# BadgerTechnologies/navigation

Measured on NVIDIA B200. Metric: ms per updateMap+inflation @4k^2 grid; DWA trajectories scored/sec, lower is better.
Workload: dtype u8

## Files before the change

navigation_b200/csrc/costmap.cu:

```cuda
#include <algorithm>
#include <chrono>
#include <cmath>
#include <cstddef>
#include <cstdlib>
#include <cstring>
#include <limits>
#include <memory>
#include <vector>

#include "costmap_kernels.cuh"
#include "inflate_propagate.cuh"
#include "mirror_kernels.cuh"

namespace navgpu {

struct Pt {
  double x, y;
};

static double dist2d(double x0, double y0, double x1, double y1) { return hypot(x1 - x0, y1 - y0); }
static double distance_to_line(double pX, double pY, double x0, double y0, double x1, double y1) {
  double A = pX - x0, B = pY - y0, C = x1 - x0, D = y1 - y0;
  double dot = A * C + B * D, len_sq = C * C + D * D, param = dot / len_sq;
  double xx, yy;
// ... 271 lines not shown
  const uint16_t* rank = nullptr;
  const uint8_t* cost = nullptr;
  int max_blocks = 0;
};

int propagate_max_blocks(int device, int R, int* out, size_t* smem_set) {
  const size_t smem = propagate_smem(R);
  if (smem > 200 * 1024) return fail(NAVGPU_ERR_UNSUPPORTED, "propagation tables for R=%d need %zu B of shared memory", R, smem);
  if (smem > *smem_set) {
    NAVGPU_CUDA(cudaFuncSetAttribute(k_inflate_propagate, cudaFuncAttributeMaxDynamicSharedMemorySize, (int)smem));
    *smem_set = smem;
  }
  int per_sm = 0, sms = 0;
  NAVGPU_CUDA(cudaOccupancyMaxActiveBlocksPerMultiprocessor(&per_sm, k_inflate_propagate, kPThreads, smem));
  NAVGPU_CUDA(cudaDeviceGetAttribute(&sms, cudaDevAttrMultiProcessorCount, device));
  if (per_sm < 1) return fail(NAVGPU_ERR_UNSUPPORTED, "k_inflate_propagate does not fit an SM for R=%d", R);
  *out = per_sm * sms;
  return NAVGPU_OK;
}

int launch_propagate(const UpdateArgs& a, const uint16_t* seeds, const PropBuffers& pb, cudaStream_t stream) {
  PropArgs pa;
  pa.master = a.master;
  pa.sx = a.sx; pa.sy = a.sy; pa.pitch = a.pitch;
  pa.win = a.win;
  pa.R = a.R;
  pa.seeds = reinterpret_cast<const uint32_t*>(seeds);
  pa.state = pb.state;
  pa.rank = pb.rank;
  pa.cost = pb.cost;
  pa.ctl = pb.ctl;
  pa.list[0] = pb.list[0];
  pa.list[1] = pb.list[1];
  const long long cells = (long long)a.pitch * a.sy;
  const int blocks = (int)std::max<long long>(1, std::min<long long>(cells / 8192, pb.max_blocks));
  NAVGPU_CUDA(cudaMemsetAsync(pb.ctl, 0, sizeof(PropCtl), stream));
  NAVGPU_CUDA(cudaMemsetAsync(reinterpret_cast<char*>(pb.ctl) + offsetof(PropCtl, kmin), 0xff, sizeof(pb.ctl->kmin), stream));
  void* args[] = {&pa};
  NAVGPU_CUDA(cudaLaunchCooperativeKernel((const void*)k_inflate_propagate, dim3(blocks), dim3(kPThreads), args,
                                          propagate_smem(a.R), stream));
  NAVGPU_LAUNCHED(1);
  return NAVGPU_OK;
}

struct TileFlags {
  unsigned* ready = nullptr;
  unsigned epoch = 0;
  unsigned long long* trace = nullptr;
  unsigned* done = nullptr;
  bool* handed_over = nullptr;
};
static_assert(kMirrorInflateTileW == kITX && kMirrorInflateTileH == kITY, "k_mirror_diff waits for k_inflate's tiles");

int launch_sweep(const UpdateArgs& a, uint16_t* seeds, cudaStream_t stream, bool force_generic, cudaEvent_t ev_mid = nullptr,
                 const PropBuffers* prop = nullptr, const TileFlags* flags = nullptr) {
  const int R = a.R;
  if ((R <= 31 && !force_generic) || (prop && R > 0)) {
    MergeSeedArgs m;
    m.master = a.master;
    m.sx = a.sx; m.sy = a.sy; m.pitch = a.pitch;
    m.def = a.def;
    m.do_reset = a.do_reset;
    m.win = a.win;
    m.ml = a.ml;
    m.R = R;
    m.seeds = seeds;
    m.early = a.early; m.ex0 = a.ex0; m.exn = a.exn; m.ey0 = a.ey0; m.eyn = a.eyn;
    m.obst_flag = a.obst_flag; m.obst_epoch = a.obst_epoch;
    m.trace = flags ? flags->trace : nullptr;
    m.lean = a.ml.n >= 1 && a.ml.n <= 2 && a.ml.policy[0] == NAVGPU_TRUE_OVERWRITE &&
             (a.ml.n == 1 || a.ml.policy[1] == NAVGPU_MAX || a.ml.policy[1] == NAVGPU_OVERWRITE) && !getenv("NAVGPU_NO_LEAN_MERGE");
    if (R > 0 && !seeds) return fail(NAVGPU_ERR_INVALID, "seed bitmask missing");
    dim3 block(kMSGroupsX, kMSRowsY);
    dim3 grid((a.pitch + kMSGroupsX * 16 - 1) / (kMSGroupsX * 16), (a.sy + kMSTileH - 1) / kMSTileH);
    const bool handover = flags && flags->ready && a.early && R > 0 && !(prop && R > 0) && !ev_mid;
    if (handover) { m.ready = flags->ready; m.epoch = flags->epoch; }
    if (a.ml.n > 0 || a.do_reset || R > 0) {
      NAVGPU_CUDA(launch_pdl(k_merge_seed, grid, block, 0, stream, m));
      NAVGPU_LAUNCHED(1);
    }
    if (ev_mid) cudaEventRecord(ev_mid, stream);
    if (prop && R > 0) return launch_propagate(a, seeds, *prop, stream);
    if (R > 0) {
      InflateArgs ia;
      ia.master = a.master;
      ia.sx = a.sx; ia.sy = a.sy; ia.pitch = a.pitch;
      ia.win = a.win;
      ia.R = R;
      ia.reach2 = a.reach2;
      ia.cost_d2 = a.cost_d2;
      ia.seeds = reinterpret_cast<const uint32_t*>(seeds);
      if (handover) {
        ia.ready = flags->ready; ia.epoch = flags->epoch; ia.ready_pitch = (int)grid.x;
        ia.done = flags->done;
        if (flags->handed_over) *flags->handed_over = flags->done != nullptr;
      }
      ia.trace = flags ? flags->trace : nullptr;
      dim3 igrid((a.sx + kITX - 1) / kITX, (a.sy + kITY - 1) / kITY);
      const int reach = (int)sqrtf((float)a.reach2 + 0.5f);
      ia.reach = reach;
      if (reach <= 12) NAVGPU_CUDA(launch_pdl(k_inflate<12>, igrid, dim3(kIThreads), 0, stream, ia));
      else if (reach <= 20) NAVGPU_CUDA(launch_pdl(k_inflate<20>, igrid, dim3(kIThreads), 0, stream, ia));
      else NAVGPU_CUDA(launch_pdl(k_inflate<31>, igrid, dim3(kIThreads), 0, stream, ia));
      NAVGPU_LAUNCHED(1);
    }
    return NAVGPU_OK;
  }
  size_t smem = update_costs_smem(R);
  if (smem > 200 * 1024) return fail(NAVGPU_ERR_UNSUPPORTED, "cell inflation radius %d needs %zu B of shared memory", R, smem);
  if (smem > 48 * 1024)
    NAVGPU_CUDA(cudaFuncSetAttribute(k_update_costs, cudaFuncAttributeMaxDynamicSharedMemorySize, (int)smem));
  dim3 grid((a.sx + kTX - 1) / kTX, (a.sy + kTY - 1) / kTY);
  k_update_costs<<<grid, kUpdateThreads, smem, stream>>>(a);
  NAVGPU_LAUNCHED(1);
  return NAVGPU_OK;
}

int ensure_seeds(uint16_t** seeds, size_t* cap, unsigned pitch, unsigned sy, cudaStream_t stream) {
  const size_t need = size_t(seed_pitch16(pitch)) * sy * sizeof(uint16_t);
  if (*seeds && need <= *cap) return NAVGPU_OK;
  if (*seeds) cudaFree(*seeds);
  *seeds = nullptr;
  NAVGPU_CUDA(cudaMalloc(seeds, need));
  NAVGPU_CUDA(cudaMemsetAsync(*seeds, 0, need, stream));
  *cap = need;
  return NAVGPU_OK;
}

int ensure_prop(navgpu_costmap* h, const Layer& L, PropBuffers* pb) {
  if (!h->d_prop_state) {
    NAVGPU_CUDA(cudaMalloc(&h->d_prop_state, 3 * h->bytes() * sizeof(uint32_t)));
    NAVGPU_CUDA(cudaMalloc(&h->d_prop_ctl, sizeof(PropCtl)));
  }
  NAVGPU_TRY(propagate_max_blocks(h->device, (int)L.tables.R, &h->prop_max_blocks, &h->prop_smem_set));
  pb->state = h->d_prop_state;
  pb->list[0] = h->d_prop_state + h->bytes();
  pb->list[1] = h->d_prop_state + 2 * h->bytes();
  pb->ctl = h->d_prop_ctl;
  pb->rank = L.d_rank;
  pb->cost = L.d_cost2d;
  pb->max_blocks = h->prop_max_blocks;
  return NAVGPU_OK;
}

struct EarlyBox {
  int on = 0, x0 = 0, xn = 0, y0 = 0, yn = 0;
  const unsigned* flag = nullptr;
  unsigned epoch = 0;
};

int launch_update(navgpu_costmap* h, const MergeLayers& ml, int do_reset, int R, const uint8_t* cost_d2, int reach2 = 0,
                  const Layer* infl = nullptr, const EarlyBox* early = nullptr) {
  UpdateArgs a;
  a.early = early && early->on && do_reset ? 1 : 0;
  a.ex0 = early ? early->x0 : 0; a.exn = early ? early->xn : 0; a.ey0 = early ? early->y0 : 0; a.eyn = early ? early->yn : 0;
  if (a.early && early->flag) { a.obst_flag = early->flag; a.obst_epoch = early->epoch; }
// ... 1341 lines not shown
```

navigation_b200/csrc/costmap_kernels.cuh:

```cuda
#pragma once

#include "common.cuh"

namespace navgpu {

__device__ __forceinline__ unsigned long long trace_now() {
  unsigned long long t;
  asm volatile("mov.u64 %0, %%globaltimer;" : "=l"(t));
  return t;
}
__device__ __forceinline__ void trace_start(unsigned long long* tr, int k) {
  if (tr && (threadIdx.x | threadIdx.y) == 0) atomicMin(&tr[2 * k], trace_now());
}
__device__ __forceinline__ void trace_end(unsigned long long* tr, int k) {
  if (tr && (threadIdx.x | threadIdx.y) == 0) atomicMax(&tr[2 * k + 1], trace_now());
}
constexpr int kCtaTraceMax = 4096;
__device__ __forceinline__ void trace_cta(unsigned long long* tr, int kernel, int cta, int slot) {
  if (tr && (threadIdx.x | threadIdx.y) == 0 && cta < kCtaTraceMax) {
    unsigned long long* rec = tr + 16 + 8 * ((size_t)kernel * kCtaTraceMax + cta);
    rec[slot] = trace_now();
    if (slot == 0) {
      unsigned smid;
      asm volatile("mov.u32 %0, %%smid;" : "=r"(smid));
// ... 1042 lines not shown
  if (R > 0) {
    const int nwords = bits_pitch / 4;
    for (int item = tid; item < rows * kTX; item += kUpdateThreads) {
      const int row = item / kTX, tx = item - row * kTX;
      const uint32_t* wrow = reinterpret_cast<const uint32_t*>(bits + row * bits_pitch);
      const int p = HX + tx;
      auto word = [&](int i) -> uint32_t { return (i < 0 || i >= nwords) ? 0u : wrow[i]; };
      auto window32 = [&](int q) -> uint32_t {
        const int wi = q >> 5, sh = q & 31;
        return __funnelshift_r(word(wi), word(wi + 1), sh);
      };
      int best = 255;
      for (int base = 0; base <= R; base += 32) {
        const uint32_t right = window32(p + base);
        const uint32_t left = window32(p - base - 31);
        int d = 255;
        if (right) d = base + (__ffs(right) - 1);
        if (left) d = min(d, base + __clz(left));
        if (d != 255) { best = d; break; }
      }
      hx[item] = (uint8_t)(best <= R ? best : 255);
    }
    __syncthreads();

    const int tx = tid & (kTX - 1), half = tid / kTX;
    const int R2 = R * R;
    for (int r = half * (kTY / 2); r < (half + 1) * (kTY / 2); ++r) {
      int best = 0x7fffffff;
      const uint8_t* col = hx + (r + R) * kTX + tx;
      for (int dy = -R; dy <= R; ++dy) {
        const int h = col[dy * kTX];
        const int d2 = (h == 255) ? 0x7fffffff : h * h + dy * dy;
        best = min(best, d2);
      }
      if (best <= R2) {
        uint8_t* cell = tile + r * kTX + tx;
        *cell = inflate_combine(*cell, table[best]);
      }
    }
    __syncthreads();
  }

  for (int item = tid; item < kTX * kTY / 16; item += kUpdateThreads) {
    const int r = item / (kTX / 16), c = (item - r * (kTX / 16)) * 16;
    const int y = ty0 + r, x = tx0 + c;
    if (y < (int)a.sy && x < (int)a.pitch)
      *reinterpret_cast<uint4*>(a.master + (size_t)y * a.pitch + x) = *reinterpret_cast<const uint4*>(tile + r * kTX + c);
  }
}


constexpr int kMSGroupsX = 16, kMSRowsY = 16, kMSRowIters = 2, kMSSubTiles = 2;
constexpr int kMSTileH = kMSRowsY * kMSRowIters * kMSSubTiles;
static_assert(128 + 2 * 31 <= 256, "k_inflate: one thread per region row");
static_assert(kMSGroupsX * 16 == (int)kMarkTileW && kMSRowsY * kMSRowIters == (int)kMarkTileH, "MergeLayers::used tile");
constexpr int kITX = 64, kITY = 128, kIThreads = 256, kIMaxRows = kITY + 2 * 31;
constexpr int kIMaskWords = (kIMaxRows + 32 + 70 + 31) / 32 + 1;
constexpr int kISparseRows = 12;
constexpr uint32_t kH2Inf = 0x3000;

__host__ __device__ inline unsigned seed_pitch16(unsigned pitch) { return pitch / 16 + 4; }

struct MergeSeedArgs {
  uint8_t* master;
  unsigned sx, sy, pitch;
  uint8_t def;
  int do_reset;
  const DevWindow* win;
  MergeLayers ml;
  int R;
  uint16_t* seeds;
  int early = 0, ex0 = 0, exn = 0, ey0 = 0, eyn = 0;
  const unsigned* obst_flag = nullptr;
  unsigned obst_epoch = 0;
  unsigned* ready = nullptr;
  unsigned epoch = 0;
  unsigned long long* trace = nullptr;
  int lean = 0;
};

__device__ __forceinline__ uint32_t inc4(uint32_t x) {
  return ((x & 0x7f7f7f7fu) + 0x01010101u) ^ (x & 0x80808080u);
}

__device__ __forceinline__ uint32_t merge4(uint32_t m, uint32_t v, int policy) {
  switch (policy) {
    case NAVGPU_TRUE_OVERWRITE: return v;
    case NAVGPU_OVERWRITE: {
      const uint32_t vn = __vcmpeq4(v, 0xffffffffu);
      return (m & vn) | (v & ~vn);
    }
    case NAVGPU_MAX: {
      const uint32_t take = __vcmpltu4(inc4(m), inc4(v));
      return (v & take) | (m & ~take);
    }
    case NAVGPU_ADDITION: {
      const uint32_t vn = __vcmpeq4(v, 0xffffffffu), mn = __vcmpeq4(m, 0xffffffffu);
      uint32_t s = __vaddus4(m, v);
      const uint32_t ge = __vcmpgeu4(s, 0xfdfdfdfdu);
      s = (ge & 0xfcfcfcfcu) | (s & ~ge);
      const uint32_t r = (mn & v) | (~mn & s);
      return (vn & m) | (~vn & r);
    }
    default: return m;
  }
}

__device__ __forceinline__ uint4 merge16(uint4 m, uint4 v, int policy) {
  switch (policy) {
// ... 191 lines not shown
      trace_end(a.trace, 1);
      trace_cta(a.trace, 0, blockIdx.y * gridDim.x + blockIdx.x, 2);
      if (a.trace && touched && (threadIdx.x | threadIdx.y) == 0) atomicMax(&a.trace[6], trace_now());
      if (a.ready) {
        __syncthreads();
        if ((threadIdx.x | threadIdx.y) == 0)
          asm volatile("st.release.gpu.u32 [%0], %1;" ::"l"(a.ready + blockIdx.y * gridDim.x + blockIdx.x), "r"(a.epoch) : "memory");
      }
      if ((blockIdx.x | blockIdx.y) == 0) cudaGridDependencySynchronize();
      return;
    }
  } else {
    cudaGridDependencySynchronize();
    w = *a.win;
  }
  trace_cta(a.trace, 0, blockIdx.y * gridDim.x + blockIdx.x, 1);
  if (!w.valid) return;
  const int R = a.R;
  const int my = R > 0 ? 3 * R + kITY : 0, mx = R > 0 ? 2 * R + kITX + 32 : 0;
  if (bx0 >= w.xn + mx || bx0 + kW <= w.x0 - mx || by0 >= w.yn + my || by0 + kH <= w.y0 - my) return;
  const int sx0 = max(0, w.x0 - R), sxn = min((int)a.sx, w.xn + R);
  const int sy0 = max(0, w.y0 - R), syn = min((int)a.sy, w.yn + R);
  const int x = bx0 + threadIdx.x * 16;
  if (a.lean && bx0 >= w.x0 && bx0 + kW <= w.xn && by0 >= w.y0 && by0 + kH <= w.yn) {
    merge_seed_lean<false>(a, x, by0);
  } else {
    for (int sub = 0; sub < kMSSubTiles; ++sub) {
      constexpr int kSH = kMSRowsY * kMSRowIters;
      const int sy_0 = by0 + sub * kSH;
      if (sy_0 >= (int)a.sy || sy_0 >= w.yn + my || sy_0 + kSH <= w.y0 - my) continue;
      const bool interior = bx0 >= w.x0 && bx0 + kW <= w.xn && sy_0 >= w.y0 && sy_0 + kSH <= w.yn;
      unsigned used_mask = 0xffffffffu;
      for (int l = 0; l < a.ml.n; ++l)
        if (a.ml.used[l] && a.ml.used[l][(blockIdx.y * kMSSubTiles + sub) * gridDim.x + blockIdx.x] == 0) used_mask &= ~(1u << l);
      if (interior) {
        merge_seed_items<true>(a, w, x, sy_0, sx0, sxn, sy0, syn, used_mask);
      } else if (x < (int)a.pitch) {
        merge_seed_items<false>(a, w, x, sy_0, sx0, sxn, sy0, syn, used_mask);
      }
    }
  }
  trace_end(a.trace, 1);
  trace_cta(a.trace, 0, blockIdx.y * gridDim.x + blockIdx.x, 2);
  if (a.trace && a.early && bx0 < a.exn && bx0 + kW > a.ex0 && by0 < a.eyn && by0 + kH > a.ey0 && (threadIdx.x | threadIdx.y) == 0)
    atomicMax(&a.trace[6], trace_now());
  if (a.ready) {
    __syncthreads();
    if ((threadIdx.x | threadIdx.y) == 0)
      asm volatile("st.release.gpu.u32 [%0], %1;" ::"l"(a.ready + blockIdx.y * gridDim.x + blockIdx.x), "r"(a.epoch) : "memory");
  }
  if (a.early && (blockIdx.x | blockIdx.y) == 0) cudaGridDependencySynchronize();
}

struct Dy2Table {
  uint32_t v[8 + 2 * 31][8];
  constexpr Dy2Table() : v() {
    for (int p = 0; p < 8 + 2 * 31; ++p)
      for (int k = 0; k < 8; ++k) v[p][k] = (uint32_t)((p - 31 - k) * (p - 31 - k)) * 0x10001u;
  }
};
__constant__ Dy2Table c_dy2 = Dy2Table();

__device__ __forceinline__ int smem_fetch_add(int* p, int v) {
  int old;
  asm volatile("atom.shared.add.s32 %0, [%1], %2;" : "=r"(old) : "r"((unsigned)__cvta_generic_to_shared(p)), "r"(v) : "memory");
  return old;
}

__device__ __forceinline__ uint32_t ldg_u16(unsigned long long addr) {
  uint32_t v;
  asm volatile("ld.global.u16 %0, [%1];" : "=r"(v) : "l"(addr) : "memory");
  return v;
}
__device__ __forceinline__ void stg_u16(unsigned long long addr, uint32_t v) {
  asm volatile("st.global.u16 [%0], %1;" ::"l"(addr), "r"(v) : "memory");
}

struct InflateArgs {
  uint8_t* master;
  unsigned sx, sy, pitch;
  const DevWindow* win;
  int R;
  int reach2;
  int reach;
  const uint8_t* cost_d2;
  const uint32_t* seeds;
  const unsigned* ready = nullptr;
  unsigned epoch = 0;
  int ready_pitch = 0;
  unsigned* done = nullptr;
  unsigned long long* trace = nullptr;
};

template <int RMAX>
__device__ __forceinline__ void inflate_tile(const InflateArgs& a) {
  constexpr int kRows = kITY + 2 * RMAX;
  __shared__ __align__(16) uint32_t pbits[kRows * 4];
  __shared__ __align__(16) uint32_t h2[kRows * (kITX / 2)];
  uint32_t* const sbits = h2;
  __shared__ uint32_t rowmask[kIMaskWords];
  __shared__ uint32_t dupmask[kIMaskWords];
  __shared__ __align__(4) uint8_t canon[(kRows + 3) & ~3];
  __shared__ uint8_t rowlist[kRows];
  __shared__ int n_seeded;
  __shared__ int next_group;
  __shared__ __align__(16) uint8_t table[((RMAX + 1) * (RMAX + 1) + 1 + 15) & ~15];
  const int tx0 = blockIdx.x * kITX, ty0 = blockIdx.y * kITY;
  const unsigned* my_flag = nullptr;
  unsigned flag_seen = 0;
  cudaTriggerProgrammaticLaunchCompletion();
  trace_start(a.trace, 2);
  trace_cta(a.trace, 1, blockIdx.y * gridDim.x + blockIdx.x, 0);
  if (a.ready) {
    constexpr int kMW = kMSGroupsX * 16, kMH = kMSTileH;
    const int mx0 = max(0, tx0 - 32) / kMW, mx1 = min((int)a.pitch - 1, tx0 + kITX + 31) / kMW;
    const int my0 = max(0, ty0 - a.R) / kMH, my1 = min((int)a.sy - 1, ty0 + kITY + a.R - 1) / kMH;
    const int nx = mx1 - mx0 + 1, n = nx * (my1 - my0 + 1);
    if ((int)threadIdx.x < n) {
      my_flag = a.ready + (my0 + (int)threadIdx.x / nx) * a.ready_pitch + mx0 + (int)threadIdx.x % nx;
      asm volatile("ld.acquire.gpu.u32 %0, [%1];" : "=r"(flag_seen) : "l"(my_flag) : "memory");
    }
  }
  {
    const int zw = (a.reach2 + 1) >> 2;
    for (int i = threadIdx.x; i <= zw; i += kIThreads) {
      uint32_t v = reinterpret_cast<const uint32_t*>(a.cost_d2)[i];
      if (i == zw) v &= ~(0xffu << (8 * ((a.reach2 + 1) & 3)));
      reinterpret_cast<uint32_t*>(table)[i] = v;
    }
  }
  if (a.ready) {
    if (my_flag) {
      while (flag_seen != a.epoch) {
        __nanosleep(32);
        asm volatile("ld.acquire.gpu.u32 %0, [%1];" : "=r"(flag_seen) : "l"(my_flag) : "memory");
      }
    }
    __syncthreads();
    if (a.trace && threadIdx.x == 0) {
      atomicMin(&a.trace[7], trace_now());
      atomicMax(&a.trace[8], trace_now());
    }
    trace_cta(a.trace, 1, blockIdx.y * gridDim.x + blockIdx.x, 1);
  } else {
    cudaGridDependencySynchronize();
    const DevWindow w = *a.win;
    trace_cta(a.trace, 1, blockIdx.y * gridDim.x + blockIdx.x, 1);
    if (!w.valid) return;
    const int R = a.R;
    if (tx0 >= w.xn + 2 * R || tx0 + kITX <= w.x0 - 2 * R || ty0 >= w.yn + 2 * R || ty0 + kITY <= w.y0 - 2 * R) return;
  }
  const int R = a.reach;
  const int rows = kITY + 2 * R;
  const int tid = threadIdx.x, lane = tid & 31, warp = tid >> 5;
  const unsigned sp32 = seed_pitch16(a.pitch) / 2;

  int any = 0;
  {
    constexpr int NI = (kRows * 4 + kIThreads - 1) / kIThreads;
    uint32_t v[NI];
#pragma unroll
    for (int k = 0; k < NI; ++k) {
      const int i = tid + k * kIThreads, gy = ty0 - R + (i >> 2);
      v[k] = 0;
      if (i < rows * 4 && gy >= 0 && gy < (int)a.sy) v[k] = __ldcg(&a.seeds[(size_t)gy * sp32 + (tx0 >> 5) + (i & 3)]);
    }
    if (tid < kIMaskWords) rowmask[tid] = dupmask[tid] = 0;
    if (tid == 0) n_seeded = next_group = 0;
#pragma unroll
    for (int k = 0; k < NI; ++k) {
      const int i = tid + k * kIThreads;
      if (i < rows * 4) sbits[i] = v[k];
      any |= v[k] != 0;
    }
  }
  if (!__syncthreads_or(any)) {
    trace_end(a.trace, 2);
    trace_cta(a.trace, 1, blockIdx.y * gridDim.x + blockIdx.x, 2);
    return;
  }
  trace_cta(a.trace, 1, blockIdx.y * gridDim.x + blockIdx.x, 4);

  {
    const uint4* sb4 = reinterpret_cast<const uint4*>(sbits);
    auto pruned = [&](int r) -> uint4 {
      uint4 c = sb4[r];
      if ((c.x | c.y | c.z | c.w) != 0 && r > 0 && r + 1 < rows) {
        const uint4 u = sb4[r - 1], d = sb4[r + 1];
        const uint32_t kx = (c.x << 1) & ((c.x >> 1) | (c.y << 31)) & u.x & d.x;
        const uint32_t ky = ((c.y << 1) | (c.x >> 31)) & ((c.y >> 1) | (c.z << 31)) & u.y & d.y;
        const uint32_t kz = ((c.z << 1) | (c.y >> 31)) & ((c.z >> 1) | (c.w << 31)) & u.z & d.z;
        const uint32_t kw = ((c.w << 1) | (c.z >> 31)) & (c.w >> 1) & u.w & d.w;
        c.x &= ~kx; c.y &= ~ky; c.z &= ~kz; c.w &= ~kw;
      }
      c.x &= ~(0xffffffffu >> R);
      c.w &= (1u << R) - 1u;
      return c;
    };
    const int r = tid;
    bool seeded = false, dup = false;
    if (r < rows) {
      const uint4 k = pruned(r);
      reinterpret_cast<uint4*>(pbits)[r] = k;
      seeded = (k.x | k.y | k.z | k.w) != 0;
      if (seeded && r > 0) {
        const uint4 p = pruned(r - 1);
        dup = k.x == p.x && k.y == p.y && k.z == p.z && k.w == p.w;
      }
    }
    const uint32_t sm = __ballot_sync(0xffffffffu, seeded), dm = __ballot_sync(0xffffffffu, dup);
    const uint32_t lm = sm & ~dm;
    int base = 0;
    if (lane == 0 && sm) {
      rowmask[warp + 1] = sm;
      dupmask[warp + 1] = dm;
      if (lm) base = smem_fetch_add(&n_seeded, __popc(lm));
    }
    base = __shfl_sync(0xffffffffu, base, 0);
    if (seeded && !dup) rowlist[base + __popc(lm & ((1u << lane) - 1u))] = (uint8_t)r;
  }
  __syncthreads();
  trace_cta(a.trace, 1, blockIdx.y * gridDim.x + blockIdx.x, 5);

  {
    if (tid < rows) {
      int qq = warp;
      uint32_t z = ~dupmask[warp + 1] & (0xffffffffu >> (31 - lane));
      while (z == 0) z = ~dupmask[--qq + 1];
      canon[tid] = (uint8_t)(32 * qq + 31 - __clz(z));
    }
    const int n_rows_listed = n_seeded;
    for (int li = warp; li < n_rows_listed; li += kIThreads / 32) {
      const int r = rowlist[li];
      const uint4 W = reinterpret_cast<const uint4*>(pbits)[r];
      const uint32_t A = lane < 16 ? W.x : W.y, B = lane < 16 ? W.y : W.z, C = lane < 16 ? W.z : W.w;
      uint32_t packed = 0;
#pragma unroll
      for (int c = 0; c < 2; ++c) {
        const int sh = (2 * lane + c) & 31;
        const uint32_t right = __funnelshift_r(B, C, sh);
        const uint32_t left = __funnelshift_rc(A, B, sh + 1);
        int d = 64;
        if (right) d = __ffs(right) - 1;
        if (left) d = min(d, __clz(left));
        const uint32_t hh = d <= R ? (uint32_t)(d * d) : kH2Inf;
        packed |= hh << (16 * c);
      }
      h2[r * (kITX / 2) + lane] = packed;
    }
  }
  __syncthreads();
  trace_cta(a.trace, 1, blockIdx.y * gridDim.x + blockIdx.x, 6);

  const uint32_t R2x2 = (uint32_t)a.reach2 * 0x10001u;
  const int x = tx0 + 2 * lane;
  const bool xok = x < (int)a.sx;
  const uint32_t keep_hi = x + 1 >= (int)a.sx ? 0xff00u : 0u;
  const bool edge_tile = tx0 + kITX > (int)a.sx || ty0 + kITY > (int)a.sy;
  for (;;) {
    int g = 0;
    if (lane == 0) g = smem_fetch_add(&next_group, 1);
    g = __shfl_sync(0xffffffffu, g, 0);
    if (g >= kITY / 8) break;
    const int yr0 = g * 8;
    uint32_t acc[8];
#pragma unroll
    for (int k = 0; k < 8; ++k) acc[k] = 0x7fff7fffu;
    {
      constexpr int NJ = 8 + 2 * RMAX, NW = (NJ + 31) / 32, NB = (NJ + 7) / 8;
      const uint32_t* hb = h2 + lane;
      const uint8_t* cn = canon + yr0 + R;
      const int p0 = yr0 + R - RMAX + 32;
      const int wi = p0 >> 5, sh = p0 & 31;
      uint32_t mw[NW];
      uint32_t anyrow = 0;
      int nrows = 0;
#pragma unroll
      for (int q = 0; q < NW; ++q) {
        mw[q] = __funnelshift_r(rowmask[wi + q], rowmask[wi + q + 1], sh);
        if (q == NW - 1 && (NJ & 31) != 0) mw[q] &= (1u << (NJ & 31)) - 1u;
        const uint32_t dw = __funnelshift_r(dupmask[wi + q], dupmask[wi + q + 1], sh);
        constexpr int kBelow = RMAX + 8;
        const uint32_t below = 32 * q >= kBelow ? 0xffffffffu : (32 * q + 32 <= kBelow ? 0u : 0xffffffffu << (kBelow & 31));
        uint32_t drop = below & dw;
        if (q == 0) drop |= ((1u << RMAX) - 1u) & (dw >> 1);
        mw[q] &= ~drop;
        anyrow |= mw[q];
        nrows += __popc(mw[q]);
      }
      if (anyrow == 0) continue;
      if (nrows <= kISparseRows) {
#pragma unroll
        for (int q = 0; q < NW; ++q) {
          uint32_t m = mw[q];
          while (m) {
            const int j = __ffs(m) - 1 + 32 * q - RMAX;
            m &= m - 1;
            const uint32_t hh = hb[cn[j] * (kITX / 2)];
            const uint4* dq = reinterpret_cast<const uint4*>(c_dy2.v[j + 31]);
            const uint4 qa = dq[0], qb = dq[1];
            acc[0] = __viaddmin_u16x2(hh, qa.x, acc[0]);
            acc[1] = __viaddmin_u16x2(hh, qa.y, acc[1]);
            acc[2] = __viaddmin_u16x2(hh, qa.z, acc[2]);
            acc[3] = __viaddmin_u16x2(hh, qa.w, acc[3]);
            acc[4] = __viaddmin_u16x2(hh, qb.x, acc[4]);
            acc[5] = __viaddmin_u16x2(hh, qb.y, acc[5]);
            acc[6] = __viaddmin_u16x2(hh, qb.z, acc[6]);
            acc[7] = __viaddmin_u16x2(hh, qb.w, acc[7]);
          }
        }
      } else {
#pragma unroll
        for (int c = 0; c < NB; ++c) {
          const uint32_t bits8 = (mw[c >> 2] >> ((c & 3) * 8)) & 0xffu;
          if (bits8 == 0) continue;
#pragma unroll
          for (int b = 0; b < 8; ++b) {
            const int j = 8 * c + b - RMAX;
            if (j > 7 + RMAX) continue;
            if (bits8 & (1u << b)) {
              const uint32_t hh = hb[cn[j] * (kITX / 2)];
#pragma unroll
              for (int k = 0; k < 8; ++k) {
                const int dy = j - k;
                if (dy >= -RMAX && dy <= RMAX) acc[k] = __viaddmin_u16x2(hh, (uint32_t)(dy * dy) * 0x10001u, acc[k]);
              }
            }
          }
        }
      }
    }
    const uint32_t out_of_reach = R2x2 + 0x10001u;
    if (edge_tile) {
      const int kmax = xok ? min(8, (int)a.sy - (ty0 + yr0)) : 0;
#pragma unroll
      for (int k = 0; k < 8; ++k)
        if (k >= kmax) acc[k] = 0x7fff7fffu;
    }
    unsigned long long prow = (unsigned long long)__cvta_generic_to_global(a.master + ((size_t)(ty0 + yr0) * a.pitch + x));
    asm volatile("" : "+l"(prow));
    const uint32_t keep_hi4 = keep_hi * 0x10001u;
#pragma unroll
    for (int half = 0; half < 2; ++half) {
      uint32_t d2[4], cur[4];
#pragma unroll
      for (int q = 0; q < 4; ++q) {
        const int k = 4 * half + q;
        d2[q] = __vminu2(acc[k], out_of_reach);
        cur[q] = 0;
        if (d2[q] != out_of_reach) cur[q] = ldg_u16(prow + (unsigned long long)((uint32_t)k * a.pitch));
      }
      if (d2[0] == out_of_reach && d2[1] == out_of_reach && d2[2] == out_of_reach && d2[3] == out_of_reach) continue;
      uint32_t old4[2], out[2];
#pragma unroll
      for (int pr = 0; pr < 2; ++pr) {
        const uint32_t da = d2[2 * pr], db = d2[2 * pr + 1];
        const uint32_t c = ((uint32_t)table[da & 0xffffu] | ((uint32_t)table[da >> 16] << 8) |
                            ((uint32_t)table[db & 0xffffu] << 16) | ((uint32_t)table[db >> 16] << 24)) & ~keep_hi4;
        old4[pr] = cur[2 * pr] | (cur[2 * pr + 1] << 16);
        out[pr] = __vmaxu4(old4[pr], c);
        d2[2 * pr] = c;
      }
      if ((__vcmpeq4(old4[0], 0xffffffffu) | __vcmpeq4(old4[1], 0xffffffffu)) != 0) {
#pragma unroll
        for (int pr = 0; pr < 2; ++pr) {
          const uint32_t c = d2[2 * pr];
          out[pr] -= __vcmpeq4(old4[pr], 0xffffffffu) & __vcmpgeu4(c, 0xfdfdfdfdu) & ~c;
        }
      }
#pragma unroll
      for (int pr = 0; pr < 2; ++pr) {
        const int k = 4 * half + 2 * pr;
        const uint32_t diff = out[pr] ^ old4[pr];
        if (diff & 0xffffu) stg_u16(prow + (unsigned long long)((uint32_t)k * a.pitch), out[pr]);
        if (diff >> 16) stg_u16(prow + (unsigned long long)((uint32_t)(k + 1) * a.pitch), out[pr] >> 16);
      }
    }
  }
  trace_end(a.trace, 2);
  trace_cta(a.trace, 1, blockIdx.y * gridDim.x + blockIdx.x, 2);
}

template <int RMAX>
__global__ void __launch_bounds__(kIThreads, 8) k_inflate(InflateArgs a) {
  inflate_tile<RMAX>(a);
  if (a.ready && (blockIdx.x | blockIdx.y) == 0) cudaGridDependencySynchronize();
  if (a.done) {
    __syncthreads();
    if (threadIdx.x == 0)
      asm volatile("st.release.gpu.u32 [%0], %1;" ::"l"(a.done + blockIdx.y * gridDim.x + blockIdx.x), "r"(a.epoch) : "memory");
  }
}

inline size_t update_costs_smem(int R) {
  const int HX = (R + 7) & ~7;
  const int groups = (kTX + 2 * HX) / 8;
  const int rows = kTY + 2 * R;
  const int bits_pitch = (groups + 3) & ~3;
  return (size_t)kTX * kTY + ((rows * bits_pitch + 15) & ~15) + (size_t)rows * kTX + (size_t)R * R + 1 + 16;
}

}
```

navigation_b200/csrc/mirror_kernels.cuh:

```cuda
#pragma once

#include "common.cuh"

namespace navgpu {

constexpr int kMirrorTileW = 128, kMirrorTileH = 16;
constexpr int kMirrorTileBytes = kMirrorTileW * kMirrorTileH;
constexpr int kMirrorWarps = 8;

struct MirrorCtl {
  unsigned n_changed;
  unsigned n_staged;
  DevWindow win;
  unsigned seq;
};

struct MirrorArgs {
  const uint8_t* master;
  uint8_t* shadow;
  unsigned sx, sy, pitch;
  unsigned tiles_x, tiles_y;
  unsigned capacity;
  uint8_t* stage;
  unsigned* stage_tile;
  unsigned* counters;
  MirrorCtl* ctl;
  const DevWindow* win;
  DevWindow* dirty;
  int all;
  int hx0, hxn, hy0, hyn;
  unsigned tx0, ty0, tw, th;
  uint8_t* host_direct;
  unsigned host_pitch;
  unsigned seq;
  const unsigned* inflate_done = nullptr;
  unsigned inflate_epoch = 0;
  int inflate_pitch = 0;
};
constexpr int kMirrorInflateTileW = 64, kMirrorInflateTileH = 128;

__device__ __forceinline__ void mirror_wait_word(const unsigned* p, unsigned want) {
  unsigned seen;
  for (;;) {
    asm volatile("ld.acquire.gpu.u32 %0, [%1];" : "=r"(seen) : "l"(p) : "memory");
    if (seen == want) break;
    __nanosleep(100);
  }
}

__device__ __forceinline__ bool group_differs(const uint4& a, const uint4& b, int n_valid) {
  if (n_valid >= 16) return ((a.x ^ b.x) | (a.y ^ b.y) | (a.z ^ b.z) | (a.w ^ b.w)) != 0;
  const uint32_t d[4] = {a.x ^ b.x, a.y ^ b.y, a.z ^ b.z, a.w ^ b.w};
  uint32_t any = 0;
#pragma unroll
  for (int k = 0; k < 4; ++k) {
    const int nb = min(4, max(0, n_valid - 4 * k));
    const uint32_t mask = nb >= 4 ? 0xffffffffu : ((1u << (8 * nb)) - 1u);
    any |= d[k] & mask;
  }
  return any != 0;
}

__global__ void __launch_bounds__(kMirrorWarps * 32) k_mirror_diff(MirrorArgs a) {
  __shared__ bool s_last;
  const int lane = threadIdx.x & 31, warp = threadIdx.x >> 5;
  if (a.inflate_done) {
    if (lane == 0) mirror_wait_word(a.inflate_done, a.inflate_epoch);
    __syncwarp();
  } else {
    cudaGridDependencySynchronize();
  }
  const unsigned local = blockIdx.x * kMirrorWarps + warp;
  const unsigned n_tiles = a.tiles_x * a.tiles_y;
  const unsigned tile = local < a.tw * a.th ? (a.ty0 + local / a.tw) * a.tiles_x + a.tx0 + local % a.tw : n_tiles;
  int rx0 = 0, rxn = (int)a.sx, ry0 = 0, ryn = (int)a.sy;
  if (!a.all) {
    const DevWindow d = *a.dirty;
    if (d.valid) {
      rx0 = max(d.x0, a.hx0); rxn = min(d.xn, a.hxn); ry0 = max(d.y0, a.hy0); ryn = min(d.yn, a.hyn);
    } else {
      rxn = ryn = 0;
    }
  }
  const unsigned tx_ = tile % a.tiles_x, ty_ = tile / a.tiles_x;
  const bool in_region = (int)(tx_ * kMirrorTileW) < rxn && (int)((tx_ + 1) * kMirrorTileW) > rx0 &&
                         (int)(ty_ * kMirrorTileH) < ryn && (int)((ty_ + 1) * kMirrorTileH) > ry0;
  if (tile < n_tiles && in_region) {
    const unsigned tx = tx_, ty = ty_;
    if (a.inflate_done) {
      if (lane < kMirrorTileW / kMirrorInflateTileW) {
        const int ix = (int)(tx * kMirrorTileW) / kMirrorInflateTileW + lane, iy = (int)(ty * kMirrorTileH) / kMirrorInflateTileH;
        if (ix < a.inflate_pitch) mirror_wait_word(a.inflate_done + iy * a.inflate_pitch + ix, a.inflate_epoch);
// ... 69 lines not shown
```

Measured before the change: 0.04098.

## Widen inflate tiles to 128 columns with four columns per lane

Doubles the k_inflate tile width to 128 and the block to 512 threads. Each lane now handles four columns, with uint2 h2 loads and u32 global read-modify-writes in place of u16. Row groups shrink from 8 to 4 rows, and h2 moves to dynamic shared memory with an opt-in attribute. The aim is to cut halo overhead per tile and make the memory accesses wider, at the cost of more shared memory per block, lower occupancy (launch bounds 4), an extra __syncthreads, and changed handover tile granularity for the mirror kernel.

```diff
diff --git a/navigation_b200/csrc/costmap.cu b/navigation_b200/csrc/costmap.cu
--- a/navigation_b200/csrc/costmap.cu
+++ b/navigation_b200/csrc/costmap.cu
@@ -347,6 +347,18 @@
 };
 static_assert(kMirrorInflateTileW == kITX && kMirrorInflateTileH == kITY, "k_mirror_diff waits for k_inflate's tiles");
 
+int allow_inflate_smem() {
+  static std::atomic<bool> done_for_device[64] = {};
+  int dev = 0;
+  NAVGPU_CUDA(cudaGetDevice(&dev));
+  if (dev >= 0 && dev < 64 && done_for_device[dev].load(std::memory_order_acquire)) return NAVGPU_OK;
+  NAVGPU_CUDA(cudaFuncSetAttribute(k_inflate<12>, cudaFuncAttributeMaxDynamicSharedMemorySize, (int)inflate_h2_bytes(12)));
+  NAVGPU_CUDA(cudaFuncSetAttribute(k_inflate<20>, cudaFuncAttributeMaxDynamicSharedMemorySize, (int)inflate_h2_bytes(20)));
+  NAVGPU_CUDA(cudaFuncSetAttribute(k_inflate<31>, cudaFuncAttributeMaxDynamicSharedMemorySize, (int)inflate_h2_bytes(31)));
+  if (dev >= 0 && dev < 64) done_for_device[dev].store(true, std::memory_order_release);
+  return NAVGPU_OK;
+}
+
 int launch_sweep(const UpdateArgs& a, uint16_t* seeds, cudaStream_t stream, bool force_generic, cudaEvent_t ev_mid = nullptr,
                  const PropBuffers* prop = nullptr, const TileFlags* flags = nullptr) {
   const int R = a.R;
@@ -394,9 +406,10 @@
       dim3 igrid((a.sx + kITX - 1) / kITX, (a.sy + kITY - 1) / kITY);
       const int reach = (int)sqrtf((float)a.reach2 + 0.5f);
       ia.reach = reach;
-      if (reach <= 12) NAVGPU_CUDA(launch_pdl(k_inflate<12>, igrid, dim3(kIThreads), 0, stream, ia));
-      else if (reach <= 20) NAVGPU_CUDA(launch_pdl(k_inflate<20>, igrid, dim3(kIThreads), 0, stream, ia));
-      else NAVGPU_CUDA(launch_pdl(k_inflate<31>, igrid, dim3(kIThreads), 0, stream, ia));
+      NAVGPU_TRY(allow_inflate_smem());
+      if (reach <= 12) NAVGPU_CUDA(launch_pdl(k_inflate<12>, igrid, dim3(kIThreads), inflate_h2_bytes(12), stream, ia));
+      else if (reach <= 20) NAVGPU_CUDA(launch_pdl(k_inflate<20>, igrid, dim3(kIThreads), inflate_h2_bytes(20), stream, ia));
+      else NAVGPU_CUDA(launch_pdl(k_inflate<31>, igrid, dim3(kIThreads), inflate_h2_bytes(31), stream, ia));
       NAVGPU_LAUNCHED(1);
     }
     return NAVGPU_OK;
diff --git a/navigation_b200/csrc/costmap_kernels.cuh b/navigation_b200/csrc/costmap_kernels.cuh
--- a/navigation_b200/csrc/costmap_kernels.cuh
+++ b/navigation_b200/csrc/costmap_kernels.cuh
@@ -1118,9 +1118,12 @@
 
 constexpr int kMSGroupsX = 16, kMSRowsY = 16, kMSRowIters = 2, kMSSubTiles = 2;
 constexpr int kMSTileH = kMSRowsY * kMSRowIters * kMSSubTiles;
-static_assert(128 + 2 * 31 <= 256, "k_inflate: one thread per region row");
 static_assert(kMSGroupsX * 16 == (int)kMarkTileW && kMSRowsY * kMSRowIters == (int)kMarkTileH, "MergeLayers::used tile");
-constexpr int kITX = 64, kITY = 128, kIThreads = 256, kIMaxRows = kITY + 2 * 31;
+constexpr int kITX = 128, kITY = 128, kIThreads = 512, kIMaxRows = kITY + 2 * 31;
+constexpr int kISeedWords = kITX / 32 + 2;
+constexpr int kIGroupRows = 4;
+static_assert(kIMaxRows <= kIThreads, "k_inflate: one thread per region row");
+static_assert(kITX == 4 * 32, "k_inflate: four columns per lane");
 constexpr int kIMaskWords = (kIMaxRows + 32 + 70 + 31) / 32 + 1;
 constexpr int kISparseRows = 12;
 constexpr uint32_t kH2Inf = 0x3000;
@@ -1418,11 +1421,11 @@
   if (a.early && (blockIdx.x | blockIdx.y) == 0) cudaGridDependencySynchronize();
 }
 
-struct Dy2Table {
-  uint32_t v[8 + 2 * 31][8];
+struct alignas(16) Dy2Table {
+  uint32_t v[kIGroupRows + 2 * 31][kIGroupRows];
   constexpr Dy2Table() : v() {
-    for (int p = 0; p < 8 + 2 * 31; ++p)
-      for (int k = 0; k < 8; ++k) v[p][k] = (uint32_t)((p - 31 - k) * (p - 31 - k)) * 0x10001u;
+    for (int p = 0; p < kIGroupRows + 2 * 31; ++p)
+      for (int k = 0; k < kIGroupRows; ++k) v[p][k] = (uint32_t)((p - 31 - k) * (p - 31 - k)) * 0x10001u;
   }
 };
 __constant__ Dy2Table c_dy2 = Dy2Table();
@@ -1433,13 +1436,13 @@
   return old;
 }
 
-__device__ __forceinline__ uint32_t ldg_u16(unsigned long long addr) {
+__device__ __forceinline__ uint32_t ldg_u32(unsigned long long addr) {
   uint32_t v;
-  asm volatile("ld.global.u16 %0, [%1];" : "=r"(v) : "l"(addr) : "memory");
+  asm volatile("ld.global.u32 %0, [%1];" : "=r"(v) : "l"(addr) : "memory");
   return v;
 }
-__device__ __forceinline__ void stg_u16(unsigned long long addr, uint32_t v) {
-  asm volatile("st.global.u16 [%0], %1;" ::"l"(addr), "r"(v) : "memory");
+__device__ __forceinline__ void stg_u32(unsigned long long addr, uint32_t v) {
+  asm volatile("st.global.u32 [%0], %1;" ::"l"(addr), "r"(v) : "memory");
 }
 
 struct InflateArgs {
@@ -1458,11 +1461,14 @@
   unsigned long long* trace = nullptr;
 };
 
+__host__ __device__ constexpr size_t inflate_h2_bytes(int rmax) { return (size_t)(kITY + 2 * rmax) * (kITX / 2) * 4; }
+
 template <int RMAX>
 __device__ __forceinline__ void inflate_tile(const InflateArgs& a) {
   constexpr int kRows = kITY + 2 * RMAX;
-  __shared__ __align__(16) uint32_t pbits[kRows * 4];
-  __shared__ __align__(16) uint32_t h2[kRows * (kITX / 2)];
+  constexpr int kSW = kISeedWords;
+  __shared__ __align__(16) uint32_t pbits[kRows * kSW];
+  extern __shared__ __align__(16) uint32_t h2[];
   uint32_t* const sbits = h2;
   __shared__ uint32_t rowmask[kIMaskWords];
   __shared__ uint32_t dupmask[kIMaskWords];
@@ -1523,20 +1529,20 @@
 
   int any = 0;
   {
-    constexpr int NI = (kRows * 4 + kIThreads - 1) / kIThreads;
+    constexpr int NI = (kRows * kSW + kIThreads - 1) / kIThreads;
     uint32_t v[NI];
 #pragma unroll
     for (int k = 0; k < NI; ++k) {
-      const int i = tid + k * kIThreads, gy = ty0 - R + (i >> 2);
+      const int i = tid + k * kIThreads, row = i / kSW, gy = ty0 - R + row;
       v[k] = 0;
-      if (i < rows * 4 && gy >= 0 && gy < (int)a.sy) v[k] = __ldcg(&a.seeds[(size_t)gy * sp32 + (tx0 >> 5) + (i & 3)]);
+      if (i < rows * kSW && gy >= 0 && gy < (int)a.sy) v[k] = __ldcg(&a.seeds[(size_t)gy * sp32 + (tx0 >> 5) + (i - row * kSW)]);
     }
     if (tid < kIMaskWords) rowmask[tid] = dupmask[tid] = 0;
     if (tid == 0) n_seeded = next_group = 0;
 #pragma unroll
     for (int k = 0; k < NI; ++k) {
       const int i = tid + k * kIThreads;
-      if (i < rows * 4) sbits[i] = v[k];
+      if (i < rows * kSW) sbits[i] = v[k];
       any |= v[k] != 0;
     }
   }
@@ -1548,31 +1554,55 @@
   trace_cta(a.trace, 1, blockIdx.y * gridDim.x + blockIdx.x, 4);
 
   {
-    const uint4* sb4 = reinterpret_cast<const uint4*>(sbits);
-    auto pruned = [&](int r) -> uint4 {
-      uint4 c = sb4[r];
-      if ((c.x | c.y | c.z | c.w) != 0 && r > 0 && r + 1 < rows) {
-        const uint4 u = sb4[r - 1], d = sb4[r + 1];
-        const uint32_t kx = (c.x << 1) & ((c.x >> 1) | (c.y << 31)) & u.x & d.x;
-        const uint32_t ky = ((c.y << 1) | (c.x >> 31)) & ((c.y >> 1) | (c.z << 31)) & u.y & d.y;
-        const uint32_t kz = ((c.z << 1) | (c.y >> 31)) & ((c.z >> 1) | (c.w << 31)) & u.z & d.z;
-        const uint32_t kw = ((c.w << 1) | (c.z >> 31)) & (c.w >> 1) & u.w & d.w;
-        c.x &= ~kx; c.y &= ~ky; c.z &= ~kz; c.w &= ~kw;
-      }
-      c.x &= ~(0xffffffffu >> R);
-      c.w &= (1u << R) - 1u;
-      return c;
+    auto pruned = [&](int r, uint32_t (&c)[kSW]) {
+      const uint2* s2 = reinterpret_cast<const uint2*>(sbits + r * kSW);
+#pragma unroll
+      for (int q = 0; q < kSW / 2; ++q) {
+        const uint2 t = s2[q];
+        c[2 * q] = t.x; c[2 * q + 1] = t.y;
+      }
+      uint32_t o = 0;
+#pragma unroll
+      for (int q = 0; q < kSW; ++q) o |= c[q];
+      if (o != 0 && r > 0 && r + 1 < rows) {
+        const uint32_t* u = sbits + (r - 1) * kSW;
+        const uint32_t* d = sbits + (r + 1) * kSW;
+        uint32_t kill[kSW];
+#pragma unroll
+        for (int q = 0; q < kSW; ++q) {
+          const uint32_t left = (c[q] << 1) | (q > 0 ? c[q - 1] >> 31 : 0u);
+          const uint32_t right = (c[q] >> 1) | (q + 1 < kSW ? c[q + 1] << 31 : 0u);
+          kill[q] = left & right & u[q] & d[q];
+        }
+#pragma unroll
+        for (int q = 0; q < kSW; ++q) c[q] &= ~kill[q];
+      }
+      c[0] &= ~(0xffffffffu >> R);
+      c[kSW - 1] &= (1u << R) - 1u;
     };
     const int r = tid;
     bool seeded = false, dup = false;
+    uint32_t k[kSW];
     if (r < rows) {
-      const uint4 k = pruned(r);
-      reinterpret_cast<uint4*>(pbits)[r] = k;
-      seeded = (k.x | k.y | k.z | k.w) != 0;
-      if (seeded && r > 0) {
-        const uint4 p = pruned(r - 1);
-        dup = k.x == p.x && k.y == p.y && k.z == p.z && k.w == p.w;
-      }
+      pruned(r, k);
+      uint32_t o = 0;
+#pragma unroll
+      for (int q = 0; q < kSW / 2; ++q) {
+        reinterpret_cast<uint2*>(pbits + r * kSW)[q] = make_uint2(k[2 * q], k[2 * q + 1]);
+        o |= k[2 * q] | k[2 * q + 1];
+      }
+      seeded = o != 0;
+    }
+    __syncthreads();
+    if (seeded && r > 0) {
+      const uint2* p2 = reinterpret_cast<const uint2*>(pbits + (r - 1) * kSW);
+      uint32_t ne = 0;
+#pragma unroll
+      for (int q = 0; q < kSW / 2; ++q) {
+        const uint2 t = p2[q];
+        ne |= (k[2 * q] ^ t.x) | (k[2 * q + 1] ^ t.y);
+      }
+      dup = ne == 0;
     }
     const uint32_t sm = __ballot_sync(0xffffffffu, seeded), dm = __ballot_sync(0xffffffffu, dup);
     const uint32_t lm = sm & ~dm;
@@ -1598,43 +1628,44 @@
     const int n_rows_listed = n_seeded;
     for (int li = warp; li < n_rows_listed; li += kIThreads / 32) {
       const int r = rowlist[li];
-      const uint4 W = reinterpret_cast<const uint4*>(pbits)[r];
-      const uint32_t A = lane < 16 ? W.x : W.y, B = lane < 16 ? W.y : W.z, C = lane < 16 ? W.z : W.w;
-      uint32_t packed = 0;
-#pragma unroll
-      for (int c = 0; c < 2; ++c) {
-        const int sh = (2 * lane + c) & 31;
+      const uint32_t* W = pbits + r * kSW + (lane >> 3);
+      const uint32_t A = W[0], B = W[1], C = W[2];
+      uint32_t packed[2] = {0, 0};
+#pragma unroll
+      for (int c = 0; c < 4; ++c) {
+        const int sh = (4 * lane + c) & 31;
         const uint32_t right = __funnelshift_r(B, C, sh);
         const uint32_t left = __funnelshift_rc(A, B, sh + 1);
         int d = 64;
         if (right) d = __ffs(right) - 1;
         if (left) d = min(d, __clz(left));
         const uint32_t hh = d <= R ? (uint32_t)(d * d) : kH2Inf;
-        packed |= hh << (16 * c);
-      }
-      h2[r * (kITX / 2) + lane] = packed;
+        packed[c >> 1] |= hh << (16 * (c & 1));
+      }
+      reinterpret_cast<uint2*>(h2 + r * (kITX / 2))[lane] = make_uint2(packed[0], packed[1]);
     }
   }
   __syncthreads();
   trace_cta(a.trace, 1, blockIdx.y * gridDim.x + blockIdx.x, 6);
 
   const uint32_t R2x2 = (uint32_t)a.reach2 * 0x10001u;
-  const int x = tx0 + 2 * lane;
+  const int x = tx0 + 4 * lane;
   const bool xok = x < (int)a.sx;
-  const uint32_t keep_hi = x + 1 >= (int)a.sx ? 0xff00u : 0u;
+  const int nvalid = (int)a.sx - x;
+  const uint32_t keep = nvalid >= 4 ? 0u : 0xffffffffu << (8 * max(nvalid, 0));
   const bool edge_tile = tx0 + kITX > (int)a.sx || ty0 + kITY > (int)a.sy;
   for (;;) {
     int g = 0;
     if (lane == 0) g = smem_fetch_add(&next_group, 1);
     g = __shfl_sync(0xffffffffu, g, 0);
-    if (g >= kITY / 8) break;
-    const int yr0 = g * 8;
-    uint32_t acc[8];
-#pragma unroll
-    for (int k = 0; k < 8; ++k) acc[k] = 0x7fff7fffu;
+    if (g >= kITY / kIGroupRows) break;
+    const int yr0 = g * kIGroupRows;
+    uint32_t acc[2 * kIGroupRows];
+#pragma unroll
+    for (int k = 0; k < 2 * kIGroupRows; ++k) acc[k] = 0x7fff7fffu;
     {
-      constexpr int NJ = 8 + 2 * RMAX, NW = (NJ + 31) / 32, NB = (NJ + 7) / 8;
-      const uint32_t* hb = h2 + lane;
+      constexpr int NJ = kIGroupRows + 2 * RMAX, NW = (NJ + 31) / 32, NB = (NJ + 7) / 8;
+      const uint2* hb = reinterpret_cast<const uint2*>(h2) + lane;
       const uint8_t* cn = canon + yr0 + R;
       const int p0 = yr0 + R - RMAX + 32;
       const int wi = p0 >> 5, sh = p0 & 31;
@@ -1646,7 +1677,7 @@
         mw[q] = __funnelshift_r(rowmask[wi + q], rowmask[wi + q + 1], sh);
         if (q == NW - 1 && (NJ & 31) != 0) mw[q] &= (1u << (NJ & 31)) - 1u;
         const uint32_t dw = __funnelshift_r(dupmask[wi + q], dupmask[wi + q + 1], sh);
-        constexpr int kBelow = RMAX + 8;
+        constexpr int kBelow = RMAX + kIGroupRows;
         const uint32_t below = 32 * q >= kBelow ? 0xffffffffu : (32 * q + 32 <= kBelow ? 0u : 0xffffffffu << (kBelow & 31));
         uint32_t drop = below & dw;
         if (q == 0) drop |= ((1u << RMAX) - 1u) & (dw >> 1);
@@ -1662,17 +1693,16 @@
           while (m) {
             const int j = __ffs(m) - 1 + 32 * q - RMAX;
             m &= m - 1;
-            const uint32_t hh = hb[cn[j] * (kITX / 2)];
-            const uint4* dq = reinterpret_cast<const uint4*>(c_dy2.v[j + 31]);
-            const uint4 qa = dq[0], qb = dq[1];
-            acc[0] = __viaddmin_u16x2(hh, qa.x, acc[0]);
-            acc[1] = __viaddmin_u16x2(hh, qa.y, acc[1]);
-            acc[2] = __viaddmin_u16x2(hh, qa.z, acc[2]);
-            acc[3] = __viaddmin_u16x2(hh, qa.w, acc[3]);
-            acc[4] = __viaddmin_u16x2(hh, qb.x, acc[4]);
-            acc[5] = __viaddmin_u16x2(hh, qb.y, acc[5]);
-            acc[6] = __viaddmin_u16x2(hh, qb.z, acc[6]);
-            acc[7] = __viaddmin_u16x2(hh, qb.w, acc[7]);
+            const uint2 hh = hb[cn[j] * (kITX / 4)];
+            const uint4 dq = *reinterpret_cast<const uint4*>(c_dy2.v[j + 31]);
+            acc[0] = __viaddmin_u16x2(hh.x, dq.x, acc[0]);
+            acc[1] = __viaddmin_u16x2(hh.y, dq.x, acc[1]);
+            acc[2] = __viaddmin_u16x2(hh.x, dq.y, acc[2]);
+            acc[3] = __viaddmin_u16x2(hh.y, dq.y, acc[3]);
+            acc[4] = __viaddmin_u16x2(hh.x, dq.z, acc[4]);
+            acc[5] = __viaddmin_u16x2(hh.y, dq.z, acc[5]);
+            acc[6] = __viaddmin_u16x2(hh.x, dq.w, acc[6]);
+            acc[7] = __viaddmin_u16x2(hh.y, dq.w, acc[7]);
           }
         }
       } else {
@@ -1683,13 +1713,16 @@
 #pragma unroll
           for (int b = 0; b < 8; ++b) {
             const int j = 8 * c + b - RMAX;
-            if (j > 7 + RMAX) continue;
+            if (j > kIGroupRows - 1 + RMAX) continue;
             if (bits8 & (1u << b)) {
-              const uint32_t hh = hb[cn[j] * (kITX / 2)];
-#pragma unroll
-              for (int k = 0; k < 8; ++k) {
+              const uint2 hh = hb[cn[j] * (kITX / 4)];
+#pragma unroll
+              for (int k = 0; k < kIGroupRows; ++k) {
                 const int dy = j - k;
-                if (dy >= -RMAX && dy <= RMAX) acc[k] = __viaddmin_u16x2(hh, (uint32_t)(dy * dy) * 0x10001u, acc[k]);
+                if (dy >= -RMAX && dy <= RMAX) {
+                  acc[2 * k] = __viaddmin_u16x2(hh.x, (uint32_t)(dy * dy) * 0x10001u, acc[2 * k]);
+                  acc[2 * k + 1] = __viaddmin_u16x2(hh.y, (uint32_t)(dy * dy) * 0x10001u, acc[2 * k + 1]);
+                }
               }
             }
           }
@@ -1698,49 +1731,36 @@
     }
     const uint32_t out_of_reach = R2x2 + 0x10001u;
     if (edge_tile) {
-      const int kmax = xok ? min(8, (int)a.sy - (ty0 + yr0)) : 0;
-#pragma unroll
-      for (int k = 0; k < 8; ++k)
-        if (k >= kmax) acc[k] = 0x7fff7fffu;
+      const int kmax = xok ? min(kIGroupRows, (int)a.sy - (ty0 + yr0)) : 0;
+#pragma unroll
+      for (int k = 0; k < kIGroupRows; ++k)
+        if (k >= kmax) acc[2 * k] = acc[2 * k + 1] = 0x7fff7fffu;
     }
     unsigned long long prow = (unsigned long long)__cvta_generic_to_global(a.master + ((size_t)(ty0 + yr0) * a.pitch + x));
     asm volatile("" : "+l"(prow));
-    const uint32_t keep_hi4 = keep_hi * 0x10001u;
-#pragma unroll
-    for (int half = 0; half < 2; ++half) {
-      uint32_t d2[4], cur[4];
-#pragma unroll
-      for (int q = 0; q < 4; ++q) {
-        const int k = 4 * half + q;
-        d2[q] = __vminu2(acc[k], out_of_reach);
-        cur[q] = 0;
-        if (d2[q] != out_of_reach) cur[q] = ldg_u16(prow + (unsigned long long)((uint32_t)k * a.pitch));
-      }
-      if (d2[0] == out_of_reach && d2[1] == out_of_reach && d2[2] == out_of_reach && d2[3] == out_of_reach) continue;
-      uint32_t old4[2], out[2];
-#pragma unroll
-      for (int pr = 0; pr < 2; ++pr) {
-        const uint32_t da = d2[2 * pr], db = d2[2 * pr + 1];
-        const uint32_t c = ((uint32_t)table[da & 0xffffu] | ((uint32_t)table[da >> 16] << 8) |
-                            ((uint32_t)table[db & 0xffffu] << 16) | ((uint32_t)table[db >> 16] << 24)) & ~keep_hi4;
-        old4[pr] = cur[2 * pr] | (cur[2 * pr + 1] << 16);
-        out[pr] = __vmaxu4(old4[pr], c);
-        d2[2 * pr] = c;
-      }
-      if ((__vcmpeq4(old4[0], 0xffffffffu) | __vcmpeq4(old4[1], 0xffffffffu)) != 0) {
-#pragma unroll
-        for (int pr = 0; pr < 2; ++pr) {
-          const uint32_t c = d2[2 * pr];
-          out[pr] -= __vcmpeq4(old4[pr], 0xffffffffu) & __vcmpgeu4(c, 0xfdfdfdfdu) & ~c;
-        }
-      }
-#pragma unroll
-      for (int pr = 0; pr < 2; ++pr) {
-        const int k = 4 * half + 2 * pr;
-        const uint32_t diff = out[pr] ^ old4[pr];
-        if (diff & 0xffffu) stg_u16(prow + (unsigned long long)((uint32_t)k * a.pitch), out[pr]);
-        if (diff >> 16) stg_u16(prow + (unsigned long long)((uint32_t)(k + 1) * a.pitch), out[pr] >> 16);
-      }
+    uint32_t cur[kIGroupRows];
+    bool hit = false;
+#pragma unroll
+    for (int k = 0; k < kIGroupRows; ++k) {
+      acc[2 * k] = __vminu2(acc[2 * k], out_of_reach);
+      acc[2 * k + 1] = __vminu2(acc[2 * k + 1], out_of_reach);
+      cur[k] = 0;
+      if (acc[2 * k] != out_of_reach || acc[2 * k + 1] != out_of_reach) {
+        cur[k] = ldg_u32(prow + (unsigned long long)((uint32_t)k * a.pitch));
+        hit = true;
+      }
+    }
+    if (!hit) continue;
+#pragma unroll
+    for (int k = 0; k < kIGroupRows; ++k) {
+      const uint32_t da = acc[2 * k], db = acc[2 * k + 1];
+      const uint32_t c = ((uint32_t)table[da & 0xffffu] | ((uint32_t)table[da >> 16] << 8) |
+                          ((uint32_t)table[db & 0xffffu] << 16) | ((uint32_t)table[db >> 16] << 24)) & ~keep;
+      const uint32_t old4 = cur[k];
+      uint32_t out = __vmaxu4(old4, c);
+      const uint32_t unknown = __vcmpeq4(old4, 0xffffffffu);
+      if (unknown) out -= unknown & __vcmpgeu4(c, 0xfdfdfdfdu) & ~c;
+      if (out != old4) stg_u32(prow + (unsigned long long)((uint32_t)k * a.pitch), out);
     }
   }
   trace_end(a.trace, 2);
@@ -1748,7 +1768,7 @@
 }
 
 template <int RMAX>
-__global__ void __launch_bounds__(kIThreads, 8) k_inflate(InflateArgs a) {
+__global__ void __launch_bounds__(kIThreads, 4) k_inflate(InflateArgs a) {
   inflate_tile<RMAX>(a);
   if (a.ready && (blockIdx.x | blockIdx.y) == 0) cudaGridDependencySynchronize();
   if (a.done) {
diff --git a/navigation_b200/csrc/mirror_kernels.cuh b/navigation_b200/csrc/mirror_kernels.cuh
--- a/navigation_b200/csrc/mirror_kernels.cuh
+++ b/navigation_b200/csrc/mirror_kernels.cuh
@@ -37,7 +37,9 @@
   unsigned inflate_epoch = 0;
   int inflate_pitch = 0;
 };
-constexpr int kMirrorInflateTileW = 64, kMirrorInflateTileH = 128;
+constexpr int kMirrorInflateTileW = 128, kMirrorInflateTileH = 128;
+static_assert(kMirrorTileW % kMirrorInflateTileW == 0 && kMirrorInflateTileH % kMirrorTileH == 0,
+              "a mirror tile lies in one row of inflate tiles and covers whole ones");
 
 __device__ __forceinline__ void mirror_wait_word(const unsigned* p, unsigned want) {
   unsigned seen;
```

After: 0.03940, median of 6. 3.9% less time.
